# dellalibera/mythril

Hardware: AMD Instinct MI355X
Metric: EVM lane-steps/s (kernel 1, C2: 65,536 concrete lanes/GPU, token.sol runtime) (higher is better)
Workload: dtype u32x8 (256-bit integer); 1 GPU; C2: 65,536 concrete lanes/GPU stepping token.sol runtime (overflow.sol.o) with random calldata; lanes_per_gpu=65536, parallelism=lanes sharded x1, RCCL coverage all-gather

## Files before the change

### mythril_amd/csrc/device_state.h

```cpp
#pragma once
#include <stdint.h>

#include "../../include/mythgpu.h"

struct DevLanes {
    uint32_t n;
    uint32_t N;
    uint32_t stack_cap, mem_cap, calldata_cap, storage_cap;
    uint32_t *code_id, *pc, *sp, *msize, *depth, *status, *aux, *steps, *flags;
    uint32_t *calldata_len, *storage_count, *ret_offset, *ret_len;
    uint32_t *sha3_count, *exp_count;
    uint64_t *gas_min, *gas_max, *gas_limit;
    uint4 *stack;
    uint32_t *mem;
    uint32_t *calldata;
    uint4 *env;
    uint4 *storage;
    uint32_t trace_cap;
    uint32_t *trace_len;
    uint32_t *trace;
    uint32_t rec_cap;
    uint32_t *rec_len;
    uint32_t *rec;
    uint32_t *fent;
};

struct DevSym {
    uint32_t node_cap, const_cap;
    uint32_t *stag;
    uint4 *node;
    uint4 *cval;
    uint32_t *n_nodes, *n_consts;
    uint32_t *mtag;
    uint2 *sttag;
};

struct DevTaint {
    uint32_t obj_cap;
    const uint32_t *prog;
    const uint8_t *force;
    uint32_t *sobj;
    unsigned long long *omask;
    uint32_t *oremap;
    uint32_t *n_obj, *n_fixed, *n_atoms, *tflags;
    unsigned long long *sink, *ymask;
};

struct DevResetImage {
    const uint32_t *pc, *depth, *status, *aux, *steps, *storage_count;
    const uint64_t *gas_min, *gas_max;
    const uint4 *storage;
};

struct DevCode {
    uint32_t n_instr;
    uint32_t n_bytes;
    uint32_t n_jres;
    uint32_t op_off;
    uint32_t addr_off;
    uint32_t push_off;
    uint32_t jres_off;
    uint32_t bytes_off;
    uint32_t cov_off;
    uint32_t run_off;
    uint32_t fent_off;
    uint32_t _pad;
};

struct DevCounters {
    unsigned long long lane_steps;
    unsigned int running, halted, hooked, escaped;
};

#define MG_JRES_NONE 0xffffffffu

#define KT_SLOTS 64u
#define KT_ENTRY 32u
#define KT_STATE 24u
#define KT_BUSY 0xffffffffu
#define KT_BYTES (KT_SLOTS * KT_ENTRY * 4u)
#define KT_EPOCH_MAX 0xfffffff0u
```

### mythril_amd/csrc/lane_step.cuh

```cuda
#pragma once
#include "device_state.h"
#include "keccak.cuh"
#include "u256.cuh"
#include "../../include/mythgpu.h"

struct OpInfo {
    uint32_t gmin, gmax;
    uint32_t req;
    uint32_t valid;
};

#ifndef MG_K1_PF
#define MG_K1_PF 0
#endif
#define RUN_MAX 64u
static_assert(RUN_MAX <= 64u, "a run is read as one pre-decoded word per wave lane");
#define BIG_END (1ull << 32)
#define HUGE_GAS (1ull << 62)

typedef unsigned int v4u __attribute__((ext_vector_type(4)));
typedef __attribute__((address_space(1))) v4u g_u4;
typedef __attribute__((address_space(3))) v4u l_u4;
typedef __attribute__((address_space(3))) uint32_t l_u32;
template <class T> DEV __attribute__((address_space(1))) T *gp(T *p) {
    return (__attribute__((address_space(1))) T *)p;
}
DEV g_u4 *gv(const void *p) { return (g_u4 *)const_cast<void *>(p); }

DEV U256 ld_word(const g_u4 *base, size_t idx) {
    const v4u x = base[2 * idx], y = base[2 * idx + 1];
    U256 r;
    r.w[0] = x.x; r.w[1] = x.y; r.w[2] = x.z; r.w[3] = x.w;
    r.w[4] = y.x; r.w[5] = y.y; r.w[6] = y.z; r.w[7] = y.w;
    return r;
}
DEV U256 ld_word(const l_u4 *base, size_t idx) {
    const v4u x = base[2 * idx], y = base[2 * idx + 1];
    U256 r;
    r.w[0] = x.x; r.w[1] = x.y; r.w[2] = x.z; r.w[3] = x.w;
    r.w[4] = y.x; r.w[5] = y.y; r.w[6] = y.z; r.w[7] = y.w;
    return r;
}
DEV void st_word(g_u4 *base, size_t idx, const U256 &v) {
    base[2 * idx] = v4u{v.w[0], v.w[1], v.w[2], v.w[3]};
    base[2 * idx + 1] = v4u{v.w[4], v.w[5], v.w[6], v.w[7]};
}
#define LANE_BLOCK 256u
struct LaneView {
    const DevLanes &L;
    uint32_t lane;
    l_u4 *win_base;
    uint32_t win, tid, ws;
    l_u32 *mw_base;
    uint32_t mw;
    DEV size_t row(uint32_t r) const { return (size_t)r * L.N + lane; }
    DEV U256 gstack(uint32_t slot) const { return ld_word(gv(L.stack), row(slot)); }
    DEV void set_gstack(uint32_t slot, const U256 &v) const { st_word(gv(L.stack), row(slot), v); }
    DEV U256 wstack(uint32_t slot) const {
        const v4u x = win_base[(slot * 2u) * ws + tid];
        const v4u y = win_base[(slot * 2u + 1u) * ws + tid];
        U256 r;
        r.w[0] = x.x; r.w[1] = x.y; r.w[2] = x.z; r.w[3] = x.w;
        r.w[4] = y.x; r.w[5] = y.y; r.w[6] = y.z; r.w[7] = y.w;
        return r;
    }
    DEV void set_wstack(uint32_t slot, const U256 &v) const {
        win_base[(slot * 2u) * ws + tid] = v4u{v.w[0], v.w[1], v.w[2], v.w[3]};
        win_base[(slot * 2u + 1u) * ws + tid] = v4u{v.w[4], v.w[5], v.w[6], v.w[7]};
// ... 673 lines not shown
    const uint32_t a = T[(size_t)(n - 2u) * N], b = T[(size_t)(n - 1u) * N];
    int32_t i = (int32_t)n - 3;
    for (; i >= 1; --i)
        if (T[(size_t)i * N] == a && T[(size_t)(i + 1) * N] == b) break;
    if (i < 1) return 0u;
    const uint32_t size = n - (uint32_t)i - 2u, base = (uint32_t)i + 1u;
    uint32_t count = 2u;
    for (int32_t j = (int32_t)base - (int32_t)size; j >= 0; j -= (int32_t)size) {
        uint32_t pj = 0u, pb = 0u;
        bool eq = true;
        for (uint32_t k = 0; k <= size; ++k) {
            const uint32_t xj = k < size ? T[(size_t)((uint32_t)j + k) * N] : 0u;
            const uint32_t xb = k < size ? T[(size_t)(base + k) * N] : 0u;
            if (((xj & 0xffu) | (pj >> 8)) != ((xb & 0xffu) | (pb >> 8))) { eq = false; break; }
            pj = xj;
            pb = xb;
        }
        if (!eq) break;
        ++count;
    }
    return count;
}

__device__ __noinline__ uint64_t trace_step(uint32_t *__restrict__ trace, size_t N, uint32_t cap, uint32_t lane,
                                            uint32_t tlen, uint32_t addr, uint32_t jumpdest, uint32_t bound,
                                            uint32_t creation) {
    if (tlen >= cap) return (uint64_t)tlen | (2ull << 60);
    trace[(size_t)tlen * N + lane] = addr;
    ++tlen;
    if (!jumpdest) return tlen;
    const uint32_t count = loop_count_dev(trace + lane, N, tlen);
    const bool drop = creation ? (count > bound && count >= 128u) : count > bound;
    return (uint64_t)tlen | ((uint64_t)count << 32) | (drop ? (1ull << 60) : 0ull);
}

__device__ __forceinline__ void reset_lane(const DevLanes &L, const DevResetImage &R, uint32_t lane) {
    L.pc[lane] = R.pc[lane]; L.sp[lane] = 0; L.msize[lane] = 0; L.depth[lane] = R.depth[lane];
    L.status[lane] = R.status[lane]; L.aux[lane] = R.aux[lane]; L.steps[lane] = R.steps[lane];
    L.gas_min[lane] = R.gas_min[lane]; L.gas_max[lane] = R.gas_max[lane];
    L.sha3_count[lane] = 0; L.exp_count[lane] = 0;
    L.trace_len[lane] = 0;
    L.rec_len[lane] = 0;
    L.fent[lane] = MG_FENT_NONE;
    const uint32_t cnt = R.storage_count[lane];
    L.storage_count[lane] = cnt;
    for (uint32_t s = 0; s < cnt; ++s)
#pragma unroll
        for (int k = 0; k < 4; ++k) {
            const size_t idx = ((size_t)s * L.N + lane) * 4 + k;
            L.storage[idx] = R.storage[idx];
        }
}

#ifdef MG_K1_CLOCKS
#define CLK_BINS 262u
__device__ uint32_t g_k1_clk[4096u * CLK_BINS];
#endif

#define K1_LPW_MASK 0xffu
#define K1_REG_RUNS 0x100u
#define K1_PUSH_LDS 0x200u
#define K1_NO_KTAB 0x400u
#define K1_MW_SHIFT 16
#define K1_MW_MASK 0xffu

template <bool kLoop>
__global__ __launch_bounds__(LANE_BLOCK) void k_lane_step(DevLanes L, const DevCode *__restrict__ codes,
                                                          const uint8_t *__restrict__ a8,
                                                          const uint32_t *__restrict__ a32,
                                                          uint8_t *__restrict__ cov, uint32_t cov_on,
                                                          uint64_t m0, uint64_t m1, uint64_t m2, uint64_t m3,
                                                          uint32_t max_steps, uint32_t max_depth,
                                                          DevCounters *__restrict__ ctr,
                                                          unsigned long long *__restrict__ prof,
                                                          uint32_t win, uint32_t pd_cap, uint32_t jr_cap,
                                                          uint32_t horizon, uint32_t loop_bound,
                                                          DevResetImage R, uint32_t lpw_flags,
                                                          uint32_t *ktab, uint32_t kepoch) {
    const uint32_t lpw = lpw_flags & K1_LPW_MASK;
    const bool lds_runs_on = (lpw_flags & K1_REG_RUNS) == 0u;
    const bool push_lds = (lpw_flags & K1_PUSH_LDS) != 0u;
    const uint32_t mw = ((lpw_flags >> K1_MW_SHIFT) & K1_MW_MASK) * 8u;
    extern __shared__ __attribute__((aligned(16))) uint4 dyn[];
    l_u4 *s_win = (l_u4 *)dyn;
    const uint32_t lanes_pb = (LANE_BLOCK / 64u) * lpw;
    l_u32 *s_mw = (l_u32 *)(dyn + (size_t)win * 2u * lanes_pb);
    uint4 *s_pd = dyn + (size_t)win * 2u * lanes_pb + (size_t)mw * lanes_pb / 4u;
    uint4 *s_push = s_pd + pd_cap;
    uint16_t *s_jr = reinterpret_cast<uint16_t *>(s_push + (push_lds ? 2u * pd_cap : 0u));
    uint8_t *s_cov = reinterpret_cast<uint8_t *>(s_jr + jr_cap);
    __shared__ uint2 s_dec[256];
    __shared__ uint32_t s_code;
    __shared__ uint32_t s_prof[260];
    __shared__ uint32_t s_kc[(LANE_BLOCK / 64u) * KC_WAVE];

    const uint32_t wlane = threadIdx.x & 63u;
    const uint32_t tid = (threadIdx.x >> 6) * lpw + wlane;
    const uint32_t lane = blockIdx.x * lanes_pb + tid;
    const bool in_range = wlane < lpw && lane < L.n;
    if (R.pc != nullptr && in_range) reset_lane(L, R, lane);
    uint32_t status = in_range ? L.status[lane] : MG_HALT_STOP;
    const uint32_t my_code = in_range ? L.code_id[lane] : 0u;
    for (uint32_t i = threadIdx.x; i < 256u; i += blockDim.x) s_dec[i] = kDec[i];
    if (prof)
        for (uint32_t i = threadIdx.x; i < 260u; i += blockDim.x) s_prof[i] = 0u;
    if (threadIdx.x == 0) s_code = 0xffffffffu;
    if ((threadIdx.x & 63u) < 2u) s_kc[(threadIdx.x >> 6) * KC_WAVE + KC_E * 24u + (threadIdx.x & 63u)] = 0u;
    __syncthreads();
    if (status == MG_RUNNING) s_code = my_code;
    __syncthreads();
#ifdef MG_K1_CLOCKS
    __shared__ uint32_t s_clk[LANE_BLOCK / 64u][CLK_BINS];
    for (uint32_t i = threadIdx.x; i < (LANE_BLOCK / 64u) * CLK_BINS; i += blockDim.x) (&s_clk[0][0])[i] = 0u;
    __syncthreads();
    __shared__ uint64_t s_clk_t[LANE_BLOCK / 64u];
    __shared__ uint32_t s_clk_bin[LANE_BLOCK / 64u];
    if ((threadIdx.x & 63u) == 0u) { s_clk_t[threadIdx.x >> 6] = __builtin_amdgcn_s_memtime();
                                     s_clk_bin[threadIdx.x >> 6] = 257u; }
#define CLK_MARK(next_) do { const uint64_t t_ = __builtin_amdgcn_s_memtime();                   \
        const uint64_t act_ = __ballot(1);                                                     \
        if ((threadIdx.x & 63u) == (uint32_t)__builtin_ctzll(act_)) {                           \
            const uint32_t w_ = threadIdx.x >> 6;                                              \
            s_clk[w_][s_clk_bin[w_]] += (uint32_t)(t_ - s_clk_t[w_]) + (1u << 24);             \
            s_clk_t[w_] = t_; s_clk_bin[w_] = (next_); } } while (0)
#else
#define CLK_MARK(next_) do { } while (0)
#endif
    const uint32_t bcode = s_code;
    const bool mixed = __syncthreads_or(status == MG_RUNNING && my_code != bcode);
    bool staged = false, jstaged = false;
    uint32_t ns_b = 0u, sn_b = 0u, jn_b = 0u, push_b = 0u;
    if (bcode != 0xffffffffu && !mixed) {
        const DevCode BC = codes[bcode];
        const uint32_t ns = min(BC.n_instr, pd_cap - 1u);
        if (ns > 0u) {
            for (uint32_t i = threadIdx.x; i < ns; i += blockDim.x) {
                const uint32_t op = a8[BC.op_off + i];
                const uint2 d = kDec[op];
                const uint64_t hm = op < 64u ? m0 : op < 128u ? m1 : op < 192u ? m2 : m3;
                const uint32_t hook = (uint32_t)((hm >> (op & 63u)) & 1ull);
                s_pd[i] = make_uint4(d.x, op | (d.y << 8) | pd_flags(op, d.y, hook) |
                                              ((uint32_t)a8[BC.fent_off + i] << 22),
                                     a32[BC.run_off + 2u * i], a32[BC.run_off + 2u * i + 1u]);
                s_cov[i] = 0;
            }
            if (threadIdx.x == 0 && ns == BC.n_instr)
                s_pd[ns] = make_uint4(0u, ((uint32_t)K_END << 17) | PD_SPECIAL, 0u, 0u);
            if (push_lds) {
                const uint4 *gpu4 = reinterpret_cast<const uint4 *>(a32 + BC.push_off);
                for (uint32_t i = threadIdx.x; i < 2u * ns; i += blockDim.x) s_push[i] = gpu4[i];
            }
            staged = true;
            ns_b = ns;
            sn_b = ns == BC.n_instr ? ns + 1u : ns;
            push_b = BC.push_off;
            const uint32_t jn = min(BC.n_jres, jr_cap);
            if (jn > 0u && BC.n_instr < 0xffffu) {
                for (uint32_t i = threadIdx.x; i < jn; i += blockDim.x) {
                    const uint32_t t = a32[BC.jres_off + i];
                    s_jr[i] = t == MG_JRES_NONE ? (uint16_t)0xffffu : (uint16_t)t;
                }
                jstaged = true;
                jn_b = jn;
            }
        }
        __syncthreads();
    }
    uint32_t executed = 0;
    const bool sym_lane = in_range && status == MG_RUNNING && (L.flags[lane] & (16u | 2048u)) != 0u;
    const bool run0 = status == MG_RUNNING && !sym_lane;
    const uint32_t sflag = __builtin_amdgcn_readfirstlane(staged ? 1u : 0u);
    const uint32_t jflag = __builtin_amdgcn_readfirstlane(jstaged ? 1u : 0u);
    const uint32_t ns = __builtin_amdgcn_readfirstlane(ns_b);
    const uint32_t sn = __builtin_amdgcn_readfirstlane(sn_b);
    const uint32_t jn = __builtin_amdgcn_readfirstlane(jn_b);
    const uint32_t bpush = __builtin_amdgcn_readfirstlane(push_b);
    const uint32_t psflag = (staged && push_lds) ? 1u : 0u;
#define PUSH_IMM(i_) (psflag ? ld_word((const l_u4 *)s_push, (i_)) : ld_word(gv(a32 + bpush), (i_)))
    const uint32_t stack_lim = L.stack_cap < MG_STACK_LIMIT ? L.stack_cap : MG_STACK_LIMIT;

    const LaneView V{L, lane, s_win, win, tid, lanes_pb, s_mw, mw};
    DevCode C{};
    uint32_t flags = 0, pc = 0, sp = 0, msize = 0, depth = 0, aux = 0, n_sha3 = 0, n_exp = 0;
    uint32_t tlen = 0;
    uint32_t fent = MG_FENT_NONE;
    const uint32_t loop_on = kLoop ? loop_bound : 0u;
    uint64_t txlim = 0, glim = 0, gmin = 0, gmax = 0;
    U256 T0 = u_zero(), T1 = u_zero();
    uint2 pd = make_uint2(0u, 0u);
    uint2 prun = make_uint2(0u, 0u);
    bool live = false;
    if (run0) {
        C = codes[my_code];
        flags = L.flags[lane];
        txlim = L.gas_limit[lane];
        glim = txlim < MG_MSTATE_GAS_LIMIT + 1ull ? txlim : MG_MSTATE_GAS_LIMIT + 1ull;
// ... 48 lines not shown
        const bool hk_ = (pd.y >> 31) && !(hook_ack && executed == 0u);                  \
        bool lstop_ = false;                                                              \
              \
             \
        if (loop_on && k_ != K_END && !(max_depth != 0u && depth >= max_depth) &&        \
            !(hook_ack && executed == 0u) && (hk_ || executed < lane_max)) {              \
            const uint64_t tr_ = trace_step(L.trace, L.N, L.trace_cap, lane, tlen,        \
                                            a32[C.addr_off + pc], o_ == 0x5bu, loop_bound,\
                                            creation ? 1u : 0u);                          \
            tlen = (uint32_t)tr_;                                                         \
            const uint32_t res_ = (uint32_t)(tr_ >> 60);                                  \
            if (res_ == 1u) { status = MG_LOOP_BOUND; aux = (uint32_t)(tr_ >> 32) & 0x0fffffffu; \
                              live = false; lstop_ = true; }                              \
            else if (res_ == 2u) { status = MG_ESCAPE; aux = o_ | (MG_ESC_TRACE << 8);        \
                                   live = false; lstop_ = true; }                         \
        }                                                                                 \
              \
              \
        if (!lstop_ && (hk_ || (pd.y & PD_SPECIAL) || executed >= lane_max ||             \
            (max_depth != 0u && depth >= max_depth) || (creation && (pd.y & PD_CREATION)))) { \
            uint32_t st_ = MG_RUNNING;                                                    \
            if (max_depth != 0u && depth >= max_depth) st_ = MG_DEPTH;                    \
            else if (k_ == K_END) st_ = MG_HALT_END;                                           \
            else if (hk_) { st_ = MG_HOOK; aux = o_; }                                    \
            else if (executed >= lane_max) live = false;                                  \
            else { st_ = MG_ESCAPE; aux = o_ | (MG_ESC_OPCODE << 8); }                       \
            if (st_ != MG_RUNNING) { status = st_; live = false; }                        \
        }                                                                                 \
    } while (0)

    if (live) FETCH();

    const bool runs_on = sflag && !prof && !loop_on && ((m0 | m1 | m2 | m3) == 0ull);

    for (;;) {
        CLK_MARK(260u);
        const uint64_t live_mask = __ballot(live);
        if (live_mask == 0ull) break;
        const int lead = __builtin_ctzll(live_mask);
        if (runs_on) {
            uint32_t upc = __builtin_amdgcn_readlane(pc, lead);
            asm volatile("" : "+s"(upc));
            const uint32_t rx = __builtin_amdgcn_readlane(prun.x, lead);
            const uint32_t ry = __builtin_amdgcn_readlane(prun.y, lead);
            const uint32_t rlen = rx & 0xffu;
            if (rlen >= 2u && upc + rlen <= ns) {
                const uint32_t rneed = (rx >> 8) & 0xffu, rpeak = (rx >> 16) & 0xffu;
                const uint32_t rjk = (rx >> 24) & 3u, rsimple = rjk ? rlen - 1u : rlen;
                const uint32_t rg0 = ry & 0xffffu, rg1 = ry >> 16;
                uint32_t usp = __builtin_amdgcn_readlane(sp, lead);
                asm volatile("" : "+s"(usp));
                const bool lds_run = lds_runs_on && usp >= rneed && usp + rpeak <= win &&
                                     usp + rpeak <= stack_lim;
                const bool in_run = live && pc == upc && sp >= rneed && sp + rpeak <= stack_lim &&
                                    gmin + rg0 < glim && executed + rlen <= lane_max &&
                                    (!lds_run || sp == usp);
                uint32_t ybulk = s_pd[min(upc + (threadIdx.x & 63u), pd_cap - 1u)].y;
                asm volatile("" : "+v"(ybulk));
                if ((__ballot(in_run) >> lead) & 1ull) {
                    CLK_MARK(256u);
                    if (in_run && lds_run) {
                        uint32_t s = usp;
                        if (s >= 1u) V.set_wstack(s - 1u, T0);
                        if (s >= 2u) V.set_wstack(s - 2u, T1);
                        for (uint32_t k = 0; k < rsimple; ++k) {
                            const uint32_t y = __builtin_amdgcn_readlane(ybulk, k);
                            const uint32_t rop = y & 0xffu;
                            switch ((y >> 17) & 31u) {
                            case K_PUSH:
                                V.set_wstack(s, PUSH_IMM(upc + k));
                                ++s;
                                break;
                            case K_DUP:
                                V.set_wstack(s, V.wstack(s - (rop - 0x7fu)));
                                ++s;
                                break;
                            case K_SWAP: {
                                const uint32_t d = rop - 0x8fu;
                                const U256 x = V.wstack(s - 1u), z = V.wstack(s - 1u - d);
                                V.set_wstack(s - 1u, z);
                                V.set_wstack(s - 1u - d, x);
                                break;
                            }
                            case K_POP:
                                --s;
                                break;
                            case K_ALU: {
                                const U256 a = V.wstack(s - 1u);
                                if (rop == 0x15u || rop == 0x19u) {
                                    V.set_wstack(s - 1u, alu(rop, a, a, a));
                                } else {
                                    const U256 b = V.wstack(s - 2u);
                                    V.set_wstack(s - 2u, alu(rop, a, b, b));
                                    --s;
                                }
                                break;
                            }
                            default:
                                break;
                            }
                        }
                        uint32_t nsp = s, npc = upc + rsimple, nexec = executed + rsimple;
                        uint32_t jg = 0u;
                        if (rjk) {
                            const U256 tgt = V.wstack(s - 1u);
                            const bool take = rjk == 1u || !u_iszero(V.wstack(s - 2u));
                            uint32_t idx = MG_JRES_NONE;
                            if (take && u_fits32(tgt) && tgt.w[0] < C.n_jres) {
                                if (jflag && tgt.w[0] < jn) { idx = s_jr[tgt.w[0]]; if (idx == 0xffffu) idx = MG_JRES_NONE; }
                                else idx = a32[C.jres_off + tgt.w[0]];
                            }
                            const uint32_t ty = take && idx != MG_JRES_NONE
                                                    ? (idx < sn ? s_pd[idx].y : (uint32_t)gops[idx] |
                                                                                ((uint32_t)gfent[idx] << 22))
                                                    : 0u;
                            if (!take || (idx != MG_JRES_NONE && (ty & 0xffu) == 0x5bu)) {
                                nsp = s - rjk;
                                npc = take ? idx : upc + rlen;
                                nexec = executed + rlen;
                                jg = rjk == 1u ? 8u : 10u;
                                if (rjk == 2u) ++depth;
                                const uint32_t jy = __builtin_amdgcn_readlane(ybulk, rsimple);
                                if (take ? (ty & PD_FENT) : (jy & PD_NFENT)) fent = npc;
                            }
                        }
                        T0 = nsp >= 1u ? V.wstack(nsp - 1u) : u_zero();
                        T1 = nsp >= 2u ? V.wstack(nsp - 2u) : u_zero();
                        sp = nsp;
                        pc = npc; gmin += rg0 + jg; gmax += rg1 + jg; executed = nexec;
                        FETCH();
                    } else if (in_run) {
                        for (uint32_t k = 0; k < rsimple; ++k) {
                            const uint32_t y = __builtin_amdgcn_readlane(ybulk, k);
                            const uint32_t rop = y & 0xffu;
                            switch ((y >> 17) & 31u) {
                            case K_PUSH: {
                                const U256 v = PUSH_IMM(upc + k);
                                if (sp >= 2u) V.set_stack(sp - 2u, T1);
                                T1 = T0; T0 = v; ++sp;
                                break;
                            }
                            case K_DUP: {
                                const uint32_t d = rop - 0x7fu;
                                const U256 v = d == 1u ? T0 : d == 2u ? T1 : V.stack(sp - d);
                                if (sp >= 2u) V.set_stack(sp - 2u, T1);
                                T1 = T0; T0 = v; ++sp;
                                break;
                            }
                            case K_SWAP: {
                                const uint32_t d = rop - 0x8fu;
                                if (d == 1u) {
                                    const U256 t = T0; T0 = T1; T1 = t;
                                } else {
                                    const U256 x = V.stack(sp - 1u - d);
                                    V.set_stack(sp - 1u - d, T0);
                                    T0 = x;
                                }
                                break;
                            }
                            case K_POP:
                                T0 = T1;
                                T1 = sp >= 3u ? V.stack(sp - 3u) : u_zero();
                                --sp;
                                break;
                            case K_ALU: {
                                const U256 r = alu(rop, T0, T1, T1);
                                T0 = r;
                                if (rop != 0x15u && rop != 0x19u) {
                                    T1 = sp >= 3u ? V.stack(sp - 3u) : u_zero();
                                    --sp;
                                }
                                break;
                            }
                            default:
                                break;
                            }
                        }
                        pc = upc + rsimple; gmin += rg0; gmax += rg1; executed += rsimple;
                        FETCH();
                    }
                    if (cov_on) {
                        const uint32_t wl = threadIdx.x & 63u;
                        if (wl < rlen) s_cov[upc + wl] = 1;
                    }
                    continue;
                }
            }
        }
        const uint32_t uy = __builtin_amdgcn_readlane(pd.y, lead);
        uint32_t ux = __builtin_amdgcn_readlane(pd.x, lead), uk = uy;
        asm volatile("" : "+s"(uk), "+s"(ux));
        if (!(live && pd.y == uy)) continue;

        const uint32_t op = uk & 0xffu, kind = (uk >> 17) & 31u;
#if MG_K1_PF
        const uint32_t pc_pf = pc + 1u;
        const uint4 q_pf = s_pd[min(pc_pf, sn - 1u)];
#endif
        CLK_MARK(op);
        if (cov_on) {
            if (sflag && pc < ns) s_cov[pc] = 1;
            else cov[C.cov_off + pc] = 1;
        }
        if (prof) atomicAdd(&s_prof[op], 1u);
        ++executed;

        const uint64_t ngmin = gmin + (ux & 0xffffu), ngmax = gmax + (ux >> 16);
        const bool gas_ok = ngmin < glim;
        bool ok = false;
#define PUSHV(v_) do { const U256 pv_ = (v_);                                   \
            if (sp >= 2u) V.set_stack(sp - 2u, T1);                          \
            T1 = T0; T0 = pv_; ++sp; ++pc; gmin = ngmin; gmax = ngmax; } while (0)
// ... 239 lines not shown
```

### mythril_amd/csrc/mythgpu.hip

```cpp
#include <hip/hip_runtime.h>

#include <algorithm>
#include <cstdarg>
#include <cstdio>
#include <cstring>
#include <string>
#include <vector>

#include "../../include/mythgpu.h"
#include <cstdlib>
#include <new>
#include "bv_eval.cuh"
#include "lane_step.cuh"
#include "sym_step.cuh"
#include "lane_fork.cuh"
#include "cc.h"

struct mg_ctx {
    int device = 0;
    hipStream_t stream = nullptr;
    hipEvent_t ev0 = nullptr, ev1 = nullptr;
    std::string err;
    std::vector<DevCode> codes;
    std::vector<uint8_t> a8;
    std::vector<uint32_t> a32;
    uint32_t cov_total = 0;
    DevCode *d_codes = nullptr;
    uint8_t *d_a8 = nullptr;
    uint32_t *d_a32 = nullptr;
    uint8_t *d_cov = nullptr;
    size_t cap_codes = 0, cap_a8 = 0, cap_a32 = 0, cap_cov = 0;
    mg_batch_cfg cfg{};
    bool have_lanes = false, uploaded = false, init_fresh = false;
    uint32_t loop_bound = 0;
    uint32_t lpw = 64;
    std::vector<uint8_t> code_used;
    DevLanes L{};
    DevSym S{};
    DevTaint T{};
    uint32_t *d_tprog = nullptr;
    uint8_t *d_tforce = nullptr;
    size_t cap_tforce = 0;
    std::vector<void *> lane_allocs;
    uint32_t *i_pc = nullptr, *i_depth = nullptr, *i_status = nullptr, *i_aux = nullptr,
             *i_steps = nullptr, *i_storage_count = nullptr;
    uint64_t *i_gas_min = nullptr, *i_gas_max = nullptr;
    uint4 *i_storage = nullptr;
    void *d_stage = nullptr;
    size_t stage_bytes = 0;
    uint8_t *h_xfer = nullptr;
    size_t h_xfer_bytes = 0;
    DevCounters *d_ctr = nullptr;
    uint32_t ctr_cap = 0;
    std::vector<DevCounters> h_ctr;
    DevCounters *d_ctr_multi = nullptr;
    size_t ctr_multi_cap = 0;
    std::vector<void *> retired;
    DevCounters *h_ctr_pin = nullptr;
    size_t h_ctr_pin_cap = 0;
    std::vector<void *> retired_host;
    std::vector<hipEvent_t> ev_batch;
    uint32_t *d_ktab = nullptr;
    uint32_t k_epoch = 0;
    BvState bv{};
};
// ... 230 lines not shown
                for (size_t i = 0; i < np; ++i) {
                    const uint8_t v = (a + 1 + i < n) ? code[a + 1 + i] : 0;
                    const size_t bit = 8 * (np - 1 - i);
                    pv[bit / 32] |= (uint32_t)v << (bit % 32);
                }
                const size_t present = std::min(np, n - (a + 1));
                if (present > 0) {
                    av = 0;
                    for (size_t i = 0; i < present && av != UINT64_MAX; ++i)
                        av = av >> 40 ? UINT64_MAX : (av << 8) | code[a + 1 + i];
                }
                a += np;
            }
        }
        argv.push_back(av);
        push.insert(push.end(), pv, pv + 8);
        a += 1;
    }
    std::vector<uint8_t> fent(ops.size() + 1, 0);
    if (!ops.empty()) fent[0] = 1;
    for (size_t i = 0; i + 2 < ops.size(); ++i) {
        if (ops[i] < 0x60 || ops[i] > 0x63 || ops[i + 1] != 0x14) continue;
        if (ops[i + 2] < 0x60 || ops[i + 2] > 0x7f || argv[i + 2] > 0xffffffffull) continue;
        const auto it = std::lower_bound(addrs.begin(), addrs.end(), (uint32_t)argv[i + 2]);
        if (it != addrs.end() && *it == (uint32_t)argv[i + 2]) fent[it - addrs.begin()] = 1;
    }
    for (size_t i = 0; i < ops.size(); ++i) fent[i] = (uint8_t)((fent[i] & 1u) | ((fent[i + 1] & 1u) << 1));
    DevCode dc{};
    dc.n_instr = (uint32_t)ops.size();
    dc.n_bytes = (uint32_t)n;
    dc.n_jres = dc.n_instr ? addrs.back() + 1u : 0u;
    dc.op_off = (uint32_t)ctx->a8.size();
    ctx->a8.insert(ctx->a8.end(), ops.begin(), ops.end());
    dc.bytes_off = (uint32_t)ctx->a8.size();
    ctx->a8.insert(ctx->a8.end(), code, code + n);
    dc.fent_off = (uint32_t)ctx->a8.size();
    ctx->a8.insert(ctx->a8.end(), fent.begin(), fent.begin() + ops.size());
    while (ctx->a8.size() % 16) ctx->a8.push_back(0);
    while (ctx->a32.size() % 8) ctx->a32.push_back(0);
    dc.push_off = (uint32_t)ctx->a32.size();
    ctx->a32.insert(ctx->a32.end(), push.begin(), push.end());
    dc.addr_off = (uint32_t)ctx->a32.size();
    ctx->a32.insert(ctx->a32.end(), addrs.begin(), addrs.end());
    dc.jres_off = (uint32_t)ctx->a32.size();
    {
        size_t k = 0;
        for (uint32_t tgt = 0; tgt < dc.n_jres; ++tgt) {
            while (k < addrs.size() && addrs[k] < tgt) ++k;
            ctx->a32.push_back(k < addrs.size() ? (uint32_t)k : MG_JRES_NONE);
        }
    }
    {
        const size_t ni = ops.size();
        std::vector<uint32_t> rx(ni + 1, 0u), ry(ni + 1, 0u);
        std::vector<int> need(ni + 1, 0), peak(ni + 1, 0), len(ni + 1, 0), jk(ni + 1, 0);
        std::vector<uint32_t> g0(ni + 1, 0u), g1(ni + 1, 0u);
        for (size_t i = ni; i-- > 0;) {
            const uint32_t b = ops[i];
            int req = -1, d = 0;
            if (b >= 0x60 && b <= 0x7f) { req = 0; d = 1; }
            else if (b >= 0x80 && b <= 0x8f) { req = (int)(b - 0x7f); d = 1; }
            else if (b >= 0x90 && b <= 0x9f) { req = (int)(b - 0x8e); d = 0; }
            else if (b == 0x50) { req = 1; d = -1; }
            else if (b == 0x5b) { req = 0; d = 0; }
            else if (b == 0x15 || b == 0x19) { req = 1; d = 0; }
            else if (b <= 0x03 && b >= 0x01) { req = 2; d = -1; }
            else if (b == 0x0b || (b >= 0x10 && b <= 0x1d)) { req = 2; d = -1; }
            if (b == 0x56 || b == 0x57) {
                len[i] = 1;
                need[i] = b == 0x56 ? 1 : 2;
                peak[i] = 0;
                jk[i] = b == 0x56 ? 1 : 2;
                g0[i] = g1[i] = 0u;
                rx[i] = 1u | ((uint32_t)need[i] << 8) | ((uint32_t)jk[i] << 24);
                ry[i] = 0u;
                continue;
            }
            if (req < 0) continue;
            const bool cont = len[i + 1] > 0 && len[i + 1] < RUN_MAX;
            len[i] = 1 + (cont ? len[i + 1] : 0);
            need[i] = std::max(req, (cont ? need[i + 1] : 0) - d);
            peak[i] = std::max(0, d + (cont ? peak[i + 1] : 0));
            jk[i] = cont ? jk[i + 1] : 0;
            g0[i] = t[b].gmin + (cont ? g0[i + 1] : 0u);
            g1[i] = t[b].gmax + (cont ? g1[i + 1] : 0u);
            rx[i] = (uint32_t)len[i] | ((uint32_t)need[i] << 8) | ((uint32_t)peak[i] << 16) |
                    ((uint32_t)jk[i] << 24);
            ry[i] = g0[i] | (g1[i] << 16);
        }
        dc.run_off = (uint32_t)ctx->a32.size();
        for (size_t i = 0; i < ni; ++i) { ctx->a32.push_back(rx[i]); ctx->a32.push_back(ry[i]); }
    }
    dc.cov_off = ctx->cov_total;
    ctx->cov_total += dc.n_instr + 1u;
    ctx->codes.push_back(dc);
    int rc;
    if ((rc = ensure_dev(ctx, ctx->d_codes, ctx->cap_codes, ctx->codes.size()))) return rc;
    if ((rc = ensure_dev(ctx, ctx->d_a8, ctx->cap_a8, ctx->a8.size() + 16))) return rc;
    if ((rc = ensure_dev(ctx, ctx->d_a32, ctx->cap_a32, ctx->a32.size() + 16))) return rc;
    const size_t old_cov = ctx->cap_cov;
    uint8_t *old_cov_ptr = ctx->d_cov;
    if (ctx->cov_total > ctx->cap_cov) {
        uint8_t *p = nullptr;
        const size_t ncap = std::max<size_t>(ctx->cov_total, 2 * ctx->cap_cov + 256);
        if (hipMalloc(&p, ncap) != hipSuccess) return set_err(ctx, MG_ENOMEM, "hipMalloc coverage");
        HIPX(ctx, hipMemsetAsync(p, 0, ncap, ctx->stream));
        if (old_cov_ptr) HIPX(ctx, hipMemcpyAsync(p, old_cov_ptr, old_cov, hipMemcpyDeviceToDevice, ctx->stream));
        HIPX(ctx, hipStreamSynchronize(ctx->stream));
        hipFree(old_cov_ptr);
        ctx->d_cov = p;
        ctx->cap_cov = ncap;
    }
    HIPX(ctx, hipMemcpyAsync(ctx->d_codes, ctx->codes.data(), ctx->codes.size() * sizeof(DevCode),
                             hipMemcpyHostToDevice, ctx->stream));
    HIPX(ctx, hipMemcpyAsync(ctx->d_a8, ctx->a8.data(), ctx->a8.size(), hipMemcpyHostToDevice, ctx->stream));
    HIPX(ctx, hipMemcpyAsync(ctx->d_a32, ctx->a32.data(), ctx->a32.size() * 4, hipMemcpyHostToDevice, ctx->stream));
    HIPX(ctx, hipStreamSynchronize(ctx->stream));
    *code_id = (uint32_t)(ctx->codes.size() - 1);
    return MG_OK;
}

extern "C" int mg_code_info(mg_ctx *ctx, uint32_t code_id, uint32_t *n_instr) {
    if (!ctx || code_id >= ctx->codes.size()) return set_err(ctx, MG_ENOCODE, "unknown code_id %u", code_id);
    if (n_instr) *n_instr = ctx->codes[code_id].n_instr;
    return MG_OK;
}

extern "C" int mg_code_fentries(mg_ctx *ctx, uint32_t code_id, uint8_t *out, uint32_t n) {
    if (!ctx || code_id >= ctx->codes.size()) return set_err(ctx, MG_ENOCODE, "unknown code_id %u", code_id);
    const DevCode &c = ctx->codes[code_id];
    if (!out || n != c.n_instr) return set_err(ctx, MG_EINVAL, "mg_code_fentries: need %u bytes", c.n_instr);
    std::memcpy(out, ctx->a8.data() + c.fent_off, n);
    return MG_OK;
}

extern "C" int mg_code_table(mg_ctx *ctx, uint32_t code_id, uint8_t *ops, uint32_t *addrs, uint32_t n) {
    if (!ctx || code_id >= ctx->codes.size()) return set_err(ctx, MG_ENOCODE, "unknown code_id %u", code_id);
    const DevCode &c = ctx->codes[code_id];
    if (!ops || !addrs || n != c.n_instr) return set_err(ctx, MG_EINVAL, "mg_code_table: need %u entries", c.n_instr);
    std::memcpy(ops, ctx->a8.data() + c.op_off, n);
    std::memcpy(addrs, ctx->a32.data() + c.addr_off, (size_t)n * 4);
    return MG_OK;
}

// ... 752 lines not shown
static LdsPlan lds_plan(const mg_ctx *ctx) {
    static const uint32_t MAX_WIN = 16u, MIN_WIN = 10u;
    uint32_t maxn = 0, maxj = 0;
    bool any = false;
    for (size_t k = 0; k < ctx->code_used.size() && k < ctx->codes.size(); ++k) any |= ctx->code_used[k] != 0;
    for (size_t k = 0; k < ctx->codes.size(); ++k) {
        if (any && (k >= ctx->code_used.size() || !ctx->code_used[k])) continue;
        maxn = std::max(maxn, ctx->codes[k].n_instr); maxj = std::max(maxj, ctx->codes[k].n_jres);
    }
    const size_t budget = 160u * 1024u / (64u / ctx->lpw) - 6144u;
    const size_t slot_bytes = 2u * lane_block(ctx) * 16u;
    const uint32_t win_cap = std::min<uint32_t>(MAX_WIN, ctx->L.stack_cap);
    LdsPlan p{};
    const uint32_t pd_full = (std::min<uint32_t>(maxn, 0xfffeu) + 1u + 15u) & ~15u;
    const uint32_t jr_full = (maxj + 15u) & ~15u;
    const size_t full = (size_t)pd_full * (16 + 32 + 1) + (size_t)jr_full * 2;
    if (maxn < 0xfffeu && full + (size_t)win_cap * slot_bytes <= budget) {
        p.pd_cap = pd_full; p.jr_cap = jr_full; p.push_lds = 1u;
    } else {
        const size_t min_win = std::min<uint32_t>(MIN_WIN, win_cap);
        const size_t avail = budget > min_win * slot_bytes ? budget - min_win * slot_bytes : 0;
        p.pd_cap = (uint32_t)std::min<size_t>(pd_full, (avail / 17u) & ~(size_t)15u);
        p.jr_cap = (uint32_t)std::min<size_t>(jr_full, ((avail - (size_t)p.pd_cap * 17u) / 2u) & ~(size_t)15u);
        p.push_lds = 0u;
    }
    const char *ev = getenv("MG_K1_PUSH");
    if (ev && std::string(ev) == "global") p.push_lds = 0u;
    if ((ev = getenv("MG_K1_PD_CAP")) != nullptr) {
        const uint32_t c = (uint32_t)strtoul(ev, nullptr, 10);
        if (c >= 1u && c < p.pd_cap) { p.pd_cap = c; p.push_lds = 0u; }
    }
    if ((ev = getenv("MG_K1_JR_CAP")) != nullptr) {
        const uint32_t c = (uint32_t)strtoul(ev, nullptr, 10);
        if (c < p.jr_cap) p.jr_cap = c;
    }
    const size_t code_bytes = (size_t)p.pd_cap * (16 + (p.push_lds ? 32 : 0) + 1) + (size_t)p.jr_cap * 2;
    uint32_t mwb = MEMWIN_DEFAULT;
    if ((ev = getenv("MG_K1_MEMWIN")) != nullptr) mwb = (uint32_t)strtoul(ev, nullptr, 10);
    mwb = std::min<uint32_t>(std::min<uint32_t>(mwb, ctx->L.mem_cap), 255u * 32u) & ~31u;
    const size_t lanes = lane_block(ctx);
    size_t left = budget > code_bytes ? budget - code_bytes : 0;
    const size_t min_stack = (size_t)std::min<uint32_t>(MIN_WIN, win_cap) * slot_bytes;
    while (mwb > 0u && (size_t)mwb * lanes + min_stack > left) mwb -= 32u;
    p.mw32 = mwb / 32u;
    left -= (size_t)mwb * lanes;
    p.win = (uint32_t)std::min<size_t>(win_cap, left / slot_bytes);
    p.bytes = (size_t)p.win * slot_bytes + (size_t)mwb * lanes + code_bytes + 16;
    return p;
}

static uint32_t k1_flags() {
    const char *r = getenv("MG_K1_RUNS");
    const char *t = getenv("MG_K1_KTAB");
    return ((r && std::string(r) == "reg") ? K1_REG_RUNS : 0u) | ((t && t[0] == '0' && !t[1]) ? K1_NO_KTAB : 0u);
}

static int launch_step(mg_ctx *ctx, const uint64_t hook_mask[4], uint32_t max_steps, uint32_t max_depth,
                       DevCounters *ctr, unsigned long long *prof = nullptr, uint32_t horizon = 0,
                       const DevResetImage *reset = nullptr, const LdsPlan *plan = nullptr,
                       int64_t kflags = -1) {
    const uint64_t zero[4] = {0, 0, 0, 0};
    const uint64_t *m = hook_mask ? hook_mask : zero;
    const LdsPlan P = plan ? *plan : lds_plan(ctx);
    if (ctx->loop_bound && ctx->L.trace_cap) {
        for (const DevCode &c : ctx->codes)
            if (c.n_bytes > 65536u) return set_err(ctx, MG_EINVAL, "loop bound needs codes below 64 KiB");
    }
    static bool attr_set = false;
    if (!attr_set) {
        (void)hipFuncSetAttribute((const void *)k_lane_step<false>, hipFuncAttributeMaxDynamicSharedMemorySize,
                                  160 * 1024 - 6144);
        (void)hipFuncSetAttribute((const void *)k_lane_step<true>, hipFuncAttributeMaxDynamicSharedMemorySize,
                                  160 * 1024 - 6144);
        (void)hipGetLastError();
        attr_set = true;
    }
    const uint32_t loop_bound = ctx->L.trace_cap ? ctx->loop_bound : 0u;
    if (ctr && blocks_for(ctx->L.n, lane_block(ctx)) > ctx->ctr_cap)
        return set_err(ctx, MG_EINVAL, "launch of %u blocks exceeds the %u statistics slots",
                       blocks_for(ctx->L.n, lane_block(ctx)), ctx->ctr_cap);
    if (ctx->k_epoch >= KT_EPOCH_MAX) {
        HIPX(ctx, hipMemsetAsync(ctx->d_ktab, 0, KT_BYTES, ctx->stream));
        ctx->k_epoch = 0;
    }
    ++ctx->k_epoch;
    hipLaunchKernelGGL(loop_bound ? k_lane_step<true> : k_lane_step<false>, dim3(blocks_for(ctx->L.n, lane_block(ctx))),
                       dim3(LANE_BLOCK), P.bytes, ctx->stream, ctx->L,
                       ctx->d_codes, ctx->d_a8, ctx->d_a32, ctx->d_cov, ctx->cfg.coverage ? 1u : 0u, m[0], m[1],
                       m[2], m[3], max_steps, max_depth, ctr, prof, P.win, P.pd_cap, P.jr_cap, horizon,
                       loop_bound, reset ? *reset : DevResetImage{},
                       ctx->lpw | (kflags >= 0 ? (uint32_t)kflags : k1_flags()) | (P.push_lds ? K1_PUSH_LDS : 0u) |
                       (P.mw32 << K1_MW_SHIFT), ctx->d_ktab, ctx->k_epoch);
    HIPX(ctx, hipGetLastError());
    if ((ctx->S.node || ctx->T.sobj) && !reset) {
        hipLaunchKernelGGL(k_sym_step, dim3(blocks_for(ctx->L.n)), dim3(256), 0, ctx->stream, ctx->L, ctx->S,
                           ctx->T, ctx->d_codes, ctx->d_a8, ctx->d_a32, m[0], m[1], m[2], m[3], max_steps, max_depth,
                           horizon, loop_bound, ctr, lane_block(ctx), prof);
        HIPX(ctx, hipGetLastError());
    }
    return MG_OK;
}

#ifdef MG_K1_CLOCKS
extern "C" int mg_k1_clocks(mg_ctx *ctx, uint32_t *out, size_t n) {
    if (!ctx || !out) return MG_EINVAL;
    HIPX(ctx, hipStreamSynchronize(ctx->stream));
    HIPX(ctx, hipMemcpyFromSymbol(out, HIP_SYMBOL(g_k1_clk), std::min<size_t>(n, 4096u * CLK_BINS) * 4u));
// ... 302 lines not shown
```

Measured before the change: 52.05 billion lane-steps/s.

## Let environment-push opcodes join pre-decoded straight-line runs

Builds a second run table in which environment-reading opcodes (ADDRESS, CALLER, CALLDATASIZE, CODESIZE, GAS-limit, PC, MSIZE, etc.) count as simple pushes, so bytecode runs containing them can run through the fused run executor instead of breaking back to the general dispatch loop. The kernel handles a new K_ENV case in both the LDS-stack and register-stack run paths, and marks runs containing CALLDATASIZE/CODESIZE so they are excluded during creation. An environment flag selects the old table. This adds a branchy env-word switch inside runs and doubles the run-table storage.

```diff
diff --git a/mythril_amd/csrc/device_state.h b/mythril_amd/csrc/device_state.h
--- a/mythril_amd/csrc/device_state.h
+++ b/mythril_amd/csrc/device_state.h
@@ -62,9 +62,8 @@
     uint32_t jres_off;
     uint32_t bytes_off;
     uint32_t cov_off;
-    uint32_t run_off;
+    uint32_t run_off[2];
     uint32_t fent_off;
-    uint32_t _pad;
 };
 
 struct DevCounters {
diff --git a/mythril_amd/csrc/lane_step.cuh b/mythril_amd/csrc/lane_step.cuh
--- a/mythril_amd/csrc/lane_step.cuh
+++ b/mythril_amd/csrc/lane_step.cuh
@@ -14,6 +14,7 @@
 #define MG_K1_PF 0
 #endif
 #define RUN_MAX 64u
+static_assert(RUN_MAX == runtab::RUN_LEN_MAX, "the run table is built for this length");
 static_assert(RUN_MAX <= 64u, "a run is read as one pre-decoded word per wave lane");
 #define BIG_END (1ull << 32)
 #define HUGE_GAS (1ull << 62)
@@ -793,6 +794,22 @@
         }
 }
 
+DEV U256 env_word(const LaneView &V, const DevCode &C, const uint32_t *a32, uint32_t op, uint32_t instr,
+                  uint32_t msize) {
+    switch (op) {
+    case 0x30: return V.env(0);
+    case 0x32: return V.env(2);
+    case 0x33: return V.env(1);
+    case 0x34: return V.env(3);
+    case 0x3a: return V.env(4);
+    case 0x36: return u_small(V.L.calldata_len[V.lane]);
+    case 0x38: return u_small(C.n_bytes);
+    case 0x45: return u_small(MG_MSTATE_GAS_LIMIT);
+    case 0x58: return u_small(a32[C.addr_off + instr]);
+    default: return u_small(msize);
+    }
+}
+
 #ifdef MG_K1_CLOCKS
 #define CLK_BINS 262u
 __device__ uint32_t g_k1_clk[4096u * CLK_BINS];
@@ -802,6 +819,7 @@
 #define K1_REG_RUNS 0x100u
 #define K1_PUSH_LDS 0x200u
 #define K1_NO_KTAB 0x400u
+#define K1_NO_RUNENV 0x1000u
 #define K1_MW_SHIFT 16
 #define K1_MW_MASK 0xffu
 
@@ -875,6 +893,7 @@
         const DevCode BC = codes[bcode];
         const uint32_t ns = min(BC.n_instr, pd_cap - 1u);
         if (ns > 0u) {
+            const uint32_t run_off = (lpw_flags & K1_NO_RUNENV) ? BC.run_off[1] : BC.run_off[0];
             for (uint32_t i = threadIdx.x; i < ns; i += blockDim.x) {
                 const uint32_t op = a8[BC.op_off + i];
                 const uint2 d = kDec[op];
@@ -882,7 +901,7 @@
                 const uint32_t hook = (uint32_t)((hm >> (op & 63u)) & 1ull);
                 s_pd[i] = make_uint4(d.x, op | (d.y << 8) | pd_flags(op, d.y, hook) |
                                               ((uint32_t)a8[BC.fent_off + i] << 22),
-                                     a32[BC.run_off + 2u * i], a32[BC.run_off + 2u * i + 1u]);
+                                     a32[run_off + 2u * i], a32[run_off + 2u * i + 1u]);
                 s_cov[i] = 0;
             }
             if (threadIdx.x == 0 && ns == BC.n_instr)
@@ -1037,9 +1056,10 @@
                 asm volatile("" : "+s"(usp));
                 const bool lds_run = lds_runs_on && usp >= rneed && usp + rpeak <= win &&
                                      usp + rpeak <= stack_lim;
+                const bool cre = creation && (rx & runtab::RX_CRE) != 0u;
                 const bool in_run = live && pc == upc && sp >= rneed && sp + rpeak <= stack_lim &&
                                     gmin + rg0 < glim && executed + rlen <= lane_max &&
-                                    (!lds_run || sp == usp);
+                                    (!lds_run || sp == usp) && !cre;
                 uint32_t ybulk = s_pd[min(upc + (threadIdx.x & 63u), pd_cap - 1u)].y;
                 asm volatile("" : "+v"(ybulk));
                 if ((__ballot(in_run) >> lead) & 1ull) {
@@ -1067,6 +1087,10 @@
                                 V.set_wstack(s - 1u - d, x);
                                 break;
                             }
+                            case K_ENV:
+                                V.set_wstack(s, env_word(V, C, a32, rop, upc + k, msize));
+                                ++s;
+                                break;
                             case K_POP:
                                 --s;
                                 break;
@@ -1143,6 +1167,12 @@
                                 }
                                 break;
                             }
+                            case K_ENV: {
+                                const U256 v = env_word(V, C, a32, rop, upc + k, msize);
+                                if (sp >= 2u) V.set_stack(sp - 2u, T1);
+                                T1 = T0; T0 = v; ++sp;
+                                break;
+                            }
                             case K_POP:
                                 T0 = T1;
                                 T1 = sp >= 3u ? V.stack(sp - 3u) : u_zero();
diff --git a/mythril_amd/csrc/mythgpu.hip b/mythril_amd/csrc/mythgpu.hip
--- a/mythril_amd/csrc/mythgpu.hip
+++ b/mythril_amd/csrc/mythgpu.hip
@@ -11,6 +11,7 @@
 #include <cstdlib>
 #include <new>
 #include "bv_eval.cuh"
+#include "run_table.h"
 #include "lane_step.cuh"
 #include "sym_step.cuh"
 #include "lane_fork.cuh"
@@ -347,44 +348,14 @@
     }
     {
         const size_t ni = ops.size();
-        std::vector<uint32_t> rx(ni + 1, 0u), ry(ni + 1, 0u);
-        std::vector<int> need(ni + 1, 0), peak(ni + 1, 0), len(ni + 1, 0), jk(ni + 1, 0);
-        std::vector<uint32_t> g0(ni + 1, 0u), g1(ni + 1, 0u);
-        for (size_t i = ni; i-- > 0;) {
-            const uint32_t b = ops[i];
-            int req = -1, d = 0;
-            if (b >= 0x60 && b <= 0x7f) { req = 0; d = 1; }
-            else if (b >= 0x80 && b <= 0x8f) { req = (int)(b - 0x7f); d = 1; }
-            else if (b >= 0x90 && b <= 0x9f) { req = (int)(b - 0x8e); d = 0; }
-            else if (b == 0x50) { req = 1; d = -1; }
-            else if (b == 0x5b) { req = 0; d = 0; }
-            else if (b == 0x15 || b == 0x19) { req = 1; d = 0; }
-            else if (b <= 0x03 && b >= 0x01) { req = 2; d = -1; }
-            else if (b == 0x0b || (b >= 0x10 && b <= 0x1d)) { req = 2; d = -1; }
-            if (b == 0x56 || b == 0x57) {
-                len[i] = 1;
-                need[i] = b == 0x56 ? 1 : 2;
-                peak[i] = 0;
-                jk[i] = b == 0x56 ? 1 : 2;
-                g0[i] = g1[i] = 0u;
-                rx[i] = 1u | ((uint32_t)need[i] << 8) | ((uint32_t)jk[i] << 24);
-                ry[i] = 0u;
-                continue;
-            }
-            if (req < 0) continue;
-            const bool cont = len[i + 1] > 0 && len[i + 1] < RUN_MAX;
-            len[i] = 1 + (cont ? len[i + 1] : 0);
-            need[i] = std::max(req, (cont ? need[i + 1] : 0) - d);
-            peak[i] = std::max(0, d + (cont ? peak[i + 1] : 0));
-            jk[i] = cont ? jk[i + 1] : 0;
-            g0[i] = t[b].gmin + (cont ? g0[i + 1] : 0u);
-            g1[i] = t[b].gmax + (cont ? g1[i + 1] : 0u);
-            rx[i] = (uint32_t)len[i] | ((uint32_t)need[i] << 8) | ((uint32_t)peak[i] << 16) |
-                    ((uint32_t)jk[i] << 24);
-            ry[i] = g0[i] | (g1[i] << 16);
+        uint32_t gt0[256], gt1[256];
+        for (int b = 0; b < 256; ++b) { gt0[b] = t[b].gmin; gt1[b] = t[b].gmax; }
+        for (int v = 0; v < 2; ++v) {
+            std::vector<uint32_t> rx, ry;
+            runtab::run_table(ops.data(), ni, gt0, gt1, v == 0, rx, ry);
+            dc.run_off[v] = (uint32_t)ctx->a32.size();
+            for (size_t i = 0; i < ni; ++i) { ctx->a32.push_back(rx[i]); ctx->a32.push_back(ry[i]); }
         }
-        dc.run_off = (uint32_t)ctx->a32.size();
-        for (size_t i = 0; i < ni; ++i) { ctx->a32.push_back(rx[i]); ctx->a32.push_back(ry[i]); }
     }
     dc.cov_off = ctx->cov_total;
     ctx->cov_total += dc.n_instr + 1u;
@@ -1243,7 +1214,9 @@
 static uint32_t k1_flags() {
     const char *r = getenv("MG_K1_RUNS");
     const char *t = getenv("MG_K1_KTAB");
-    return ((r && std::string(r) == "reg") ? K1_REG_RUNS : 0u) | ((t && t[0] == '0' && !t[1]) ? K1_NO_KTAB : 0u);
+    const char *e = getenv("MG_K1_RUNENV");
+    return ((r && std::string(r) == "reg") ? K1_REG_RUNS : 0u) | ((t && t[0] == '0' && !t[1]) ? K1_NO_KTAB : 0u) |
+           ((e && e[0] == '0' && !e[1]) ? K1_NO_RUNENV : 0u);
 }
 
 static int launch_step(mg_ctx *ctx, const uint64_t hook_mask[4], uint32_t max_steps, uint32_t max_depth,
diff --git a/mythril_amd/csrc/run_table.h b/mythril_amd/csrc/run_table.h
--- /dev/null
+++ b/mythril_amd/csrc/run_table.h
@@ -0,0 +1,66 @@
+#pragma once
+#include <stdint.h>
+
+#include <algorithm>
+#include <vector>
+
+namespace runtab {
+
+enum : uint32_t {
+    RUN_LEN_MAX = 64u,
+    RX_CRE = 1u << 27,
+};
+
+static inline bool env_push(uint32_t b) {
+    return b == 0x30 || (b >= 0x32 && b <= 0x34) || b == 0x36 || b == 0x38 || b == 0x3a || b == 0x45 ||
+           b == 0x58 || b == 0x59;
+}
+
+static inline bool simple_op(uint32_t b, int &req, int &d, bool env) {
+    if ((b >= 0x60 && b <= 0x7f) || (env && env_push(b))) { req = 0; d = 1; }
+    else if (b >= 0x80 && b <= 0x8f) { req = (int)(b - 0x7f); d = 1; }
+    else if (b >= 0x90 && b <= 0x9f) { req = (int)(b - 0x8e); d = 0; }
+    else if (b == 0x50) { req = 1; d = -1; }
+    else if (b == 0x5b) { req = 0; d = 0; }
+    else if (b == 0x15 || b == 0x19) { req = 1; d = 0; }
+    else if (b <= 0x03 && b >= 0x01) { req = 2; d = -1; }
+    else if (b == 0x0b || (b >= 0x10 && b <= 0x1d)) { req = 2; d = -1; }
+    else return false;
+    return true;
+}
+
+static inline void run_table(const uint8_t *ops, size_t ni, const uint32_t *gas_min, const uint32_t *gas_max,
+                             bool env, std::vector<uint32_t> &rx, std::vector<uint32_t> &ry) {
+    rx.assign(ni + 1, 0u);
+    ry.assign(ni + 1, 0u);
+    std::vector<int> need(ni + 1, 0), peak(ni + 1, 0), len(ni + 1, 0), jk(ni + 1, 0);
+    std::vector<uint32_t> g0(ni + 1, 0u), g1(ni + 1, 0u);
+    for (size_t i = ni; i-- > 0;) {
+        const uint32_t b = ops[i];
+        int req = -1, d = 0;
+        if (b == 0x56 || b == 0x57) {
+            len[i] = 1;
+            need[i] = b == 0x56 ? 1 : 2;
+            peak[i] = 0;
+            jk[i] = b == 0x56 ? 1 : 2;
+            g0[i] = g1[i] = 0u;
+            rx[i] = 1u | ((uint32_t)need[i] << 8) | ((uint32_t)jk[i] << 24);
+            ry[i] = 0u;
+            continue;
+        }
+        if (!simple_op(b, req, d, env)) continue;
+        const bool cont = len[i + 1] > 0 && len[i + 1] < (int)RUN_LEN_MAX;
+        len[i] = 1 + (cont ? len[i + 1] : 0);
+        need[i] = std::max(req, (cont ? need[i + 1] : 0) - d);
+        peak[i] = std::max(0, d + (cont ? peak[i + 1] : 0));
+        jk[i] = cont ? jk[i + 1] : 0;
+        g0[i] = gas_min[b] + (cont ? g0[i + 1] : 0u);
+        g1[i] = gas_max[b] + (cont ? g1[i + 1] : 0u);
+        rx[i] = (uint32_t)len[i] | ((uint32_t)need[i] << 8) | ((uint32_t)peak[i] << 16) |
+                ((uint32_t)jk[i] << 24) | ((b == 0x36 || b == 0x38) ? (uint32_t)RX_CRE : 0u) |
+                (cont ? rx[i + 1] & RX_CRE : 0u);
+        ry[i] = g0[i] | (g1[i] << 16);
+    }
+}
+
+}
```

Result: faster. 54.02 billion lane-steps/s (median of 6 runs) (+3.8%).
